# jianing-sun/Mask-YOLO

Hardware: AMD Instinct MI355X
Metric: images/sec fwd+bwd, 224x224 Shapes batch 32, at 1 MI355X (higher is better)
Workload: dtype f32

## Files before the change

### mask-yolo_amd/csrc/gemm_kernels.hip

```cpp
#include "myolo_common.h"

typedef float f32x16 __attribute__((ext_vector_type(16)));

#define BM 128
#define BN 128
#define BK 16
#define LDAS (BM + 2)

enum { AM_PLAIN = 0, AM_CONV3 = 1, AM_DECONV = 2 };
enum { EP_PLAIN = 0, EP_DECONV = 1, EP_DECONV_MASK = 2 };

struct GemmArgs {
    const float* A;
    const float* B;
    float* C;
    const float* bias;
    const float* scale;
    const float* shift;
    long long M;
    int N;
    int K;
    long long lda, ldb, ldc;
    int H, W;
    int Cc;
// ... 717 lines not shown

    const int lr = tid >> 5, c4 = (tid & 31) * 4;
    const int ka = ka0 + c4;
    const bool ka_ok = ka < p.K;
    int tap = 0, c0 = ka;
    if (AMODE != AM_PLAIN) { tap = ka / p.Cc; c0 = ka - tap * p.Cc; }
    const int ty = tap / 3, tx = tap - ty * 3;
    const int ky = tap >> 1, kx = tap & 1;

    long long a_base, a_end, a_row_elems;
    if (AMODE == AM_PLAIN) { a_base = ms; a_end = me; a_row_elems = p.lda; }
    else if (AMODE == AM_CONV3) {
        a_base = ms - (p.W + 1); if (a_base < 0) a_base = 0;
        a_end = me + p.W + 1; if (a_end > p.M) a_end = p.M;
        a_row_elems = p.Cc;
    } else {
        a_base = 4 * ms - 2 * p.W; if (a_base < 0) a_base = 0;
        a_end = 4 * me + 2 * p.W + 2; if (a_end > 4 * p.M) a_end = 4 * p.M;
        a_row_elems = p.Cc;
    }
    const __amdgpu_buffer_rsrc_t ra_desc = make_rsrc(p.A + a_base * a_row_elems, (a_end - a_base) * a_row_elems * 4);
    const __amdgpu_buffer_rsrc_t rb_desc = make_rsrc(p.B + ms * p.ldb, (me - ms) * p.ldb * 4);
    const bool bcol_ok = (n0 + c4) < p.N;

    long long mrow[2];
    int ry[2], rx[2];
    unsigned alin[2], blin[2];
    const unsigned a_step = (unsigned)(BK * a_row_elems) * 4u * (AMODE == AM_DECONV ? 4u : 1u);
    const unsigned b_step = (unsigned)(BK * p.ldb) * 4u;
    const unsigned two_cc = (unsigned)(2 * a_row_elems) * 4u;
    long long tapshift = 0;
    if (AMODE == AM_CONV3) tapshift = (long long)(ty - 1) * p.W + (tx - 1);
    if (AMODE == AM_DECONV) tapshift = (long long)ky * 2 * p.W + kx;
#pragma unroll
    for (int i = 0; i < 2; ++i) {
        mrow[i] = ms + lr + 8 * i;
        ry[i] = 0; rx[i] = 0;
        if (AMODE != AM_PLAIN) {
            const long long mm = mrow[i] < p.M ? mrow[i] : 0;
            const long long n_img = mm / hw;
            const int rem = (int)(mm - n_img * hw);
            ry[i] = rem / p.W;
            rx[i] = rem - ry[i] * p.W;
        }
        if (AMODE == AM_PLAIN) alin[i] = (unsigned)((mrow[i] - a_base) * a_row_elems + ka) * 4u;
        else if (AMODE == AM_CONV3) alin[i] = (unsigned)((mrow[i] + tapshift - a_base) * a_row_elems + c0) * 4u;
        else alin[i] = (unsigned)((4 * mrow[i] + tapshift - a_base) * a_row_elems + c0) * 4u;
        blin[i] = (unsigned)((mrow[i] - ms) * p.ldb + n0 + c4) * 4u;
    }

    f32x16 acc[2][2];
#pragma unroll
    for (int t = 0; t < 2; ++t)
#pragma unroll
        for (int u = 0; u < 2; ++u)
#pragma unroll
            for (int r = 0; r < 16; ++r) acc[t][u][r] = 0.f;

    float4 ra[2], rb[2];
    bool rav[2] = {false, false};
    float4 tsc = make_float4(1.f, 1.f, 1.f, 1.f), tsh = make_float4(0.f, 0.f, 0.f, 0.f);
    if (AMODE == AM_PLAIN && p.a_scale && ka_ok) { tsc = ld4(p.a_scale + ka); tsh = ld4(p.a_shift + ka); }
    auto gload = [&]() {
#pragma unroll
        for (int i = 0; i < 2; ++i) {
            const bool mv = mrow[i] < me;
            rav[i] = mv && ka_ok;
            unsigned aoff = OOB_OFF;
            if (AMODE == AM_PLAIN) {
                if (mv && ka_ok) aoff = alin[i];
            } else if (AMODE == AM_CONV3) {
                const bool v = mv && ka_ok && (unsigned)(ry[i] + ty - 1) < (unsigned)p.H && (unsigned)(rx[i] + tx - 1) < (unsigned)p.W;
                if (v) aoff = alin[i];
            } else {
                if (mv && ka_ok) aoff = alin[i] - (unsigned)rx[i] * two_cc;
            }
            ra[i] = bufld4(ra_desc, aoff);
            rb[i] = bufld4(rb_desc, (mv && bcol_ok) ? blin[i] : OOB_OFF);
            mrow[i] += BK;
            alin[i] += a_step;
            blin[i] += b_step;
            if (AMODE != AM_PLAIN) {
                int nx = rx[i] + BK;
                const int w2 = (nx >= 2 * p.W) ? 2 : ((nx >= p.W) ? 1 : 0);
                nx -= w2 * p.W;
                int ny = ry[i] + w2;
                ny = (ny >= p.H) ? ny - p.H : ny;
                rx[i] = nx; ry[i] = ny;
            }
        }
    };
    auto sstore = [&](int buf) {
        if (AMODE == AM_PLAIN && p.a_scale) {
#pragma unroll
            for (int i = 0; i < 2; ++i)
                if (rav[i]) {
                    ra[i].x = gemm_act(fmaf(ra[i].x, tsc.x, tsh.x), p.a_act); ra[i].y = gemm_act(fmaf(ra[i].y, tsc.y, tsh.y), p.a_act);
                    ra[i].z = gemm_act(fmaf(ra[i].z, tsc.z, tsh.z), p.a_act); ra[i].w = gemm_act(fmaf(ra[i].w, tsc.w, tsh.w), p.a_act);
                }
        }
#pragma unroll
        for (int i = 0; i < 2; ++i) {
            *reinterpret_cast<float4*>(&As[buf][lr + 8 * i][c4]) = ra[i];
            *reinterpret_cast<float4*>(&Bs[buf][lr + 8 * i][c4]) = rb[i];
        }
    };

    const long long nsteps = (me > ms) ? (me - ms + BK - 1) / BK : 0;
    const int half = lane >> 5, l31 = lane & 31;
    const int arow_l = wm * 64 + l31, bcol_l = wn * 64 + l31;
    if (nsteps > 0) {
        gload();
        sstore(0);
        __syncthreads();
        int cur = 0;
        for (long long st = 0; st < nsteps; ++st) {
            const bool more = st + 1 < nsteps;
            if (more) gload();
            float fa0 = As[cur][half * 8][arow_l], fa1 = As[cur][half * 8][arow_l + 32];
            float fb0 = Bs[cur][half * 8][bcol_l], fb1 = Bs[cur][half * 8][bcol_l + 32];
#pragma unroll
            for (int j = 0; j < 8; ++j) {
                float na0 = 0.f, na1 = 0.f, nb0 = 0.f, nb1 = 0.f;
                if (j < 7) {
                    const int kk = half * 8 + j + 1;
                    na0 = As[cur][kk][arow_l]; na1 = As[cur][kk][arow_l + 32];
                    nb0 = Bs[cur][kk][bcol_l]; nb1 = Bs[cur][kk][bcol_l + 32];
                }
                MFMA_STEP()
                if (j == 3 && more) sstore(cur ^ 1);
                fa0 = na0; fa1 = na1; fb0 = nb0; fb1 = nb1;
            }
            __syncthreads();
            cur ^= 1;
        }
    }
    const int nb = p.batch > 1 ? p.batch : 1;
    float* Cp = p.C + ((long long)blockIdx.y * nb + blockIdx.z) * p.K * p.N;
#pragma unroll
    for (int t = 0; t < 2; ++t)
#pragma unroll
        for (int r = 0; r < 16; ++r) {
            const int row = ka0 + wm * 64 + t * 32 + (r & 3) + 8 * (r >> 2) + 4 * half;
            if (row >= p.K) continue;
#pragma unroll
            for (int u = 0; u < 2; ++u) {
                const int col = n0 + wn * 64 + u * 32 + l31;
                if (col < p.N) Cp[(long long)row * p.N + col] = acc[t][u][r];
            }
        }
}

template <int KT, int NT>
__global__ __launch_bounds__(256) void pw_wgrad_thin(const float* __restrict__ x, const float* __restrict__ dy, float* __restrict__ part,
                                                     long long M, int Cin, int Cout, const float* __restrict__ a_scale,
                                                     const float* __restrict__ a_shift, int a_act)
{
    __shared__ float red[4][32 * 32];
    const int lane = threadIdx.x & 63, wave = threadIdx.x >> 6;
    const int half = lane >> 5, l31 = lane & 31;
    f32x16 acc[KT][NT];
#pragma unroll
    for (int a = 0; a < KT; ++a)
#pragma unroll
        for (int b = 0; b < NT; ++b)
#pragma unroll
            for (int r = 0; r < 16; ++r) acc[a][b][r] = 0.f;
    float xs[KT], xt[KT];
#pragma unroll
    for (int a = 0; a < KT; ++a) { xs[a] = a_scale ? a_scale[32 * a + l31] : 1.f; xt[a] = a_scale ? a_shift[32 * a + l31] : 0.f; }
    const long long nwaves = (long long)gridDim.x * 4;
    const long long w0 = (long long)blockIdx.x * 4 + wave;
    constexpr int RS = (KT + NT <= 3) ? 8 : 4;
    for (long long m0 = w0 * (2 * RS); m0 < M; m0 += nwaves * (2 * RS)) {
        float xa[RS][KT], yb[RS][NT];
#pragma unroll
        for (int st = 0; st < RS; ++st) {
            const long long m = m0 + 2 * st + half;
            const bool ok = m < M;
#pragma unroll
            for (int a = 0; a < KT; ++a) {
                float v = ok ? x[m * Cin + 32 * a + l31] : 0.f;
                if (a_scale && ok) v = gemm_act(fmaf(v, xs[a], xt[a]), a_act);
                xa[st][a] = v;
            }
#pragma unroll
            for (int b = 0; b < NT; ++b) yb[st][b] = ok ? dy[m * Cout + 32 * b + l31] : 0.f;
        }
#pragma unroll
        for (int st = 0; st < RS; ++st)
#pragma unroll
            for (int a = 0; a < KT; ++a)
#pragma unroll
                for (int b = 0; b < NT; ++b)
                    acc[a][b] = __builtin_amdgcn_mfma_f32_32x32x2f32(xa[st][a], yb[st][b], acc[a][b], 0, 0, 0);
    }
    float* dst = part + (long long)blockIdx.x * Cin * Cout;
#pragma unroll
    for (int a = 0; a < KT; ++a)
#pragma unroll
        for (int b = 0; b < NT; ++b) {
            __syncthreads();
#pragma unroll
            for (int r = 0; r < 16; ++r) red[wave][((r & 3) + 8 * (r >> 2) + 4 * half) * 32 + l31] = acc[a][b][r];
            __syncthreads();
            for (int e = threadIdx.x; e < 1024; e += 256) {
                const float v = (red[0][e] + red[1][e]) + (red[2][e] + red[3][e]);
                dst[(long long)(32 * a + (e >> 5)) * Cout + 32 * b + (e & 31)] = v;
            }
        }
}

__global__ __launch_bounds__(256) void partial_sum_small(const float* __restrict__ part, float* __restrict__ out, int n, int splits)
{
    __shared__ float red[4][64];
    const int e = blockIdx.x * 64 + (threadIdx.x & 63), sl = threadIdx.x >> 6;
    float s[8] = {0.f, 0.f, 0.f, 0.f, 0.f, 0.f, 0.f, 0.f};
    if (e < n) {
        int k = sl;
        for (; k + 28 < splits; k += 32) {
#pragma unroll
            for (int u = 0; u < 8; ++u) s[u] += part[(long long)(k + 4 * u) * n + e];
        }
        for (; k < splits; k += 4) s[0] += part[(long long)k * n + e];
    }
    red[sl][threadIdx.x & 63] = ((s[0] + s[1]) + (s[2] + s[3])) + ((s[4] + s[5]) + (s[6] + s[7]));
    __syncthreads();
    if (sl == 0 && e < n) out[e] = (red[0][threadIdx.x] + red[1][threadIdx.x]) + (red[2][threadIdx.x] + red[3][threadIdx.x]);
}

__global__ __launch_bounds__(256) void splitk_reduce(const float* __restrict__ part, float* __restrict__ out, long long n, int splits)
{
    const long long n4 = (n & 3) ? 0 : (n >> 2);
    long long i = (long long)blockIdx.x * blockDim.x + threadIdx.x;
    const long long stride = (long long)gridDim.x * blockDim.x;
    const float4* p4 = reinterpret_cast<const float4*>(part);
    for (; i < n4; i += stride) {
        float4 s = make_float4(0.f, 0.f, 0.f, 0.f);
        int k = 0;
        for (; k + 4 <= splits; k += 4) {
            const float4 a = p4[(long long)(k + 0) * n4 + i], b = p4[(long long)(k + 1) * n4 + i];
            const float4 c = p4[(long long)(k + 2) * n4 + i], d = p4[(long long)(k + 3) * n4 + i];
            s.x += a.x; s.y += a.y; s.z += a.z; s.w += a.w;
            s.x += b.x; s.y += b.y; s.z += b.z; s.w += b.w;
            s.x += c.x; s.y += c.y; s.z += c.z; s.w += c.w;
            s.x += d.x; s.y += d.y; s.z += d.z; s.w += d.w;
        }
        for (; k < splits; ++k) {
            const float4 a = p4[(long long)k * n4 + i];
            s.x += a.x; s.y += a.y; s.z += a.z; s.w += a.w;
        }
        reinterpret_cast<float4*>(out)[i] = s;
    }
    for (long long j = (n4 << 2) + (long long)blockIdx.x * blockDim.x + threadIdx.x; j < n; j += stride) {
        float t = 0.f;
        for (int k = 0; k < splits; ++k) t += part[(long long)k * n + j];
        out[j] = t;
    }
}

template <int EPI>
__global__ __launch_bounds__(256) void splitk_epilogue(GemmArgs p)
{
    const long long total = p.M * (long long)(p.N >> 2);
    long long i = (long long)blockIdx.x * blockDim.x + threadIdx.x;
    const long long stride = (long long)gridDim.x * blockDim.x;
    const int nq = p.N >> 2;
    const long long slab = p.M * (long long)p.N;
    const long long hw = (long long)p.H * p.W;
    for (; i < total; i += stride) {
        const long long row = i / nq;
        const int col = (int)(i - row * nq) * 4;
        float4 s = make_float4(0.f, 0.f, 0.f, 0.f);
        for (int k = 0; k < p.ksplits; ++k) {
            const float4 a = *reinterpret_cast<const float4*>(p.part + k * slab + row * p.N + col);
            s.x += a.x; s.y += a.y; s.z += a.z; s.w += a.w;
        }
        float v[4] = {s.x, s.y, s.z, s.w};
        int tap = 0, cc = col;
        if (EPI == EP_DECONV) { tap = col / p.Co; cc = col - tap * p.Co; }
#pragma unroll
        for (int e = 0; e < 4; ++e) {
            if (p.bias) v[e] += p.bias[cc + e];
            if (p.scale) { float cs, ct; col_affine(p, col + e, cs, ct); v[e] = fmaf(v[e], cs, ct); }
            v[e] = gemm_act(v[e], p.act);
        }
        float* dst;
        if (EPI == EP_PLAIN) {
            dst = p.C + row * p.ldc + col;
        } else {
            const long long n_img = row / hw;
            const int rem = (int)(row - n_img * hw);
            const int y = rem / p.W, x = rem - y * p.W;
            dst = p.C + (n_img * 4 * hw + (long long)y * 4 * p.W + 2 * x + (long long)(tap >> 1) * 2 * p.W + (tap & 1)) * p.Co + cc;
        }
        *reinterpret_cast<float4*>(dst) = make_float4(v[0], v[1], v[2], v[3]);
    }
}

__global__ void transpose_batched(const float* __restrict__ in, float* __restrict__ out, int R, int C, int nz, int reverse)
{
    __shared__ float tile[32][33];
    const int z = blockIdx.z;
    const int zi = reverse ? (nz - 1 - z) : z;
    const float* ip = in + (long long)zi * R * C;
    float* op = out + (long long)z * R * C;
    const int c0 = blockIdx.x * 32, r0 = blockIdx.y * 32;
    for (int i = threadIdx.y; i < 32; i += blockDim.y) {
        const int r = r0 + i, c = c0 + threadIdx.x;
        tile[i][threadIdx.x] = (r < R && c < C) ? ip[(long long)r * C + c] : 0.f;
    }
    __syncthreads();
    for (int i = threadIdx.y; i < 32; i += blockDim.y) {
        const int c = c0 + i, r = r0 + threadIdx.x;
        if (r < R && c < C) op[(long long)c * R + r] = tile[threadIdx.x][i];
    }
}

__global__ __launch_bounds__(256) void deconv_mask_finish(const float* __restrict__ part, const float* __restrict__ b2,
                                                          float* __restrict__ out, long long npix, int ncls, int nslabs)
{
    const long long total = npix * ncls;
    for (long long i = (long long)blockIdx.x * blockDim.x + threadIdx.x; i < total; i += (long long)gridDim.x * blockDim.x) {
        float sacc = b2[(int)(i % ncls)];
        for (int k = 0; k < nslabs; ++k) sacc += part[(long long)k * total + i];
        out[i] = 1.f / (1.f + expf(-sacc));
    }
}

static int launch_transpose(const float* in, float* out, int R, int C, int nz, int reverse, hipStream_t s)
{
    dim3 grid((C + 31) / 32, (R + 31) / 32, nz), block(32, 8);
    hipLaunchKernelGGL(transpose_batched, grid, block, 0, s, in, out, R, C, nz, reverse);
    return 0;
}

static inline long long pw_x6_min_rows() { return g_myolo_opt.pw_x6_min_rows > 0 ? g_myolo_opt.pw_x6_min_rows : 4096; }

template <int AMODE, int EPI>
static int launch_nn(const GemmArgs& a, hipStream_t s, void* sk_ws = nullptr, size_t sk_ws_bytes = 0, long long sk_max_tiles = 512,
                     int* path = nullptr)
{
    if (path) *path = 0;
    const long long tiles = cdiv64(a.M, BM) * ((a.N + BN - 1) / BN);
    if (tiles <= 0) return MYOLO_OK;
    const bool aligned = (a.N & 3) == 0 && (a.ldb & 3) == 0 && ((uintptr_t)a.A & 15) == 0 && ((uintptr_t)a.B & 15) == 0;
    const bool kfast = (AMODE == AM_PLAIN) ? ((a.K % BK) == 0 && (a.lda & 3) == 0) : ((a.Cc % BK) == 0);
    GemmArgs& am = const_cast<GemmArgs&>(a);
    am.nt = (long long)a.M * a.N * 4 > (64ll << 20);
    if (aligned && kfast && !g_myolo_opt.gemm_generic) {
        const int nk = a.K / BK;
        int splits = 1;
        if (sk_ws && tiles < sk_max_tiles && nk >= 16 && (a.N & 3) == 0 && (EPI == EP_PLAIN ? (a.ldc & 3) == 0 : (a.Co & 3) == 0) &&
            !g_myolo_opt.no_splitk) {
            splits = (int)(1024 / tiles);
            if (splits > nk / 8) splits = nk / 8;
            const size_t per = (size_t)a.M * a.N * sizeof(float);
            if ((size_t)splits * per > sk_ws_bytes) splits = (int)(sk_ws_bytes / per);
            if (splits < 2) splits = 1;
        }
        if (path) *path = splits > 1 ? splits : 1;
        if (splits > 1) {
            am.ksplits = splits;
// ... 442 lines not shown
}

static bool pw_fwd_thin_ok(long long M, int Cin, int Cout)
{
    return (Cin == 32 || Cin == 64) && Cout == 64 && M >= 8192 && !g_myolo_opt.no_trunk_fusion;
}

static int pw_fwd_thin_wgs(long long M)
{
    long long wgs = ((M + 31) / 32 + 3) / 4;
    if (wgs > 2048) wgs = 2048;
    return (int)wgs;
}

static void pw_fwd_thin_launch(const float* x, const float* in_scale, const float* in_shift, int in_act, const float* w, float* y, double* stat,
                               long long M, int Cin, int Cout, hipStream_t s, const float* o_scale = nullptr, const float* o_shift = nullptr,
                               int o_act = MYOLO_ACT_NONE)
{
    const unsigned wgs = (unsigned)pw_fwd_thin_wgs(M);
    size_t lds = (size_t)Cout * (Cin + 4) * sizeof(float);
    if (lds < (size_t)8 * Cout * sizeof(double)) lds = (size_t)8 * Cout * sizeof(double);
#define PWT(NU_, NJ_) hipLaunchKernelGGL((pw_fwd_thin_kernel<NU_, NJ_>), dim3(wgs), dim3(256), lds, s, x, w, y, stat, M, in_scale, in_shift, in_act, o_scale, o_shift, o_act)
    if (Cin == 32) PWT(2, 4);
    else PWT(2, 8);
#undef PWT
}

static bool pw_bwd_data_thin_ok(long long M, int Cin, int Cout)
{
    return (Cin == 32 || Cin == 64) && Cout <= 256 && (Cout % 8) == 0 && M >= 8192;
}


extern "C" {

int myolo_pwconv1x1_fwd(const float* x, const float* w, const float* bias, float* y,
                        int64_t M, int Cin, int Cout, void* ws, size_t ws_bytes, void* stream)
{
    MYOLO_REQUIRE(x && w && y && M > 0 && Cin > 0 && Cout > 0, "pwconv1x1_fwd: bad arguments");
    GemmArgs a = {};
    a.A = x; a.B = w; a.C = y; a.bias = bias; a.M = M; a.N = Cout; a.K = Cin;
    a.lda = Cin; a.ldb = Cout; a.ldc = Cout; a.act = MYOLO_ACT_NONE;
    if (Cout <= 64 && (Cout & 3) != 0 && (Cin & 15) == 0 && ((uintptr_t)x & 15) == 0 && !g_myolo_opt.gemm_generic) {
        if (Cin >= 512 && (Cin & 63) == 0)
            hipLaunchKernelGGL(pw_skinny_fwd_kernel<16>, dim3((unsigned)cdiv64(M, 4)), dim3(1024), 0, (hipStream_t)stream, x, w, bias, y, (long long)M, Cin, Cout);
        else
            hipLaunchKernelGGL(pw_skinny_fwd_kernel<4>, dim3((unsigned)cdiv64(M, 4)), dim3(256), 0, (hipStream_t)stream, x, w, bias, y, (long long)M, Cin, Cout);
        MYOLO_CHECK_LAUNCH();
        return MYOLO_OK;
    }
    if (!bias && pw_fwd_thin_ok(M, Cin, Cout) && (((uintptr_t)x | (uintptr_t)w | (uintptr_t)y) & 15) == 0 && !g_myolo_opt.gemm_generic) {
        pw_fwd_thin_launch(x, nullptr, nullptr, MYOLO_ACT_NONE, w, y, nullptr, M, Cin, Cout, (hipStream_t)stream);
        MYOLO_CHECK_LAUNCH();
        return MYOLO_OK;
    }
    if (pw_smallm_ok(a)) {
        pw_smallm_launch(a, (hipStream_t)stream);
        MYOLO_CHECK_LAUNCH();
        return MYOLO_OK;
    }
    launch_nn<AM_PLAIN, EP_PLAIN>(a, (hipStream_t)stream, ws, ws_bytes, 128);
    MYOLO_CHECK_LAUNCH();
    return MYOLO_OK;
}

int myolo_pwconv1x1_affine_act_fwd(const float* x, const float* w, const float* scale, const float* shift, int act, float* y,
                                   int64_t M, int Cin, int Cout, void* ws, size_t ws_bytes, void* stream)
{
    MYOLO_REQUIRE(x && w && y && scale && shift && M > 0 && Cin > 0 && Cout > 0, "pwconv1x1_affine_act_fwd: bad arguments");
    GemmArgs a = {};
    a.A = x; a.B = w; a.C = y; a.M = M; a.N = Cout; a.K = Cin;
    a.lda = Cin; a.ldb = Cout; a.ldc = Cout; a.act = act;
    a.scale = scale; a.shift = shift;
    if (pw_fwd_thin_ok(M, Cin, Cout) && (((uintptr_t)x | (uintptr_t)w | (uintptr_t)y) & 15) == 0 && !g_myolo_opt.gemm_generic) {
        pw_fwd_thin_launch(x, nullptr, nullptr, MYOLO_ACT_NONE, w, y, nullptr, M, Cin, Cout, (hipStream_t)stream, scale, shift, act);
        MYOLO_CHECK_LAUNCH();
        return MYOLO_OK;
    }
    if (pw_smallm_ok(a)) {
        pw_smallm_launch(a, (hipStream_t)stream);
        MYOLO_CHECK_LAUNCH();
        return MYOLO_OK;
    }
    launch_nn<AM_PLAIN, EP_PLAIN>(a, (hipStream_t)stream, ws, ws_bytes, 128);
    MYOLO_CHECK_LAUNCH();
    return MYOLO_OK;
}

int myolo_pwconv1x1_bwd_data(const float* dy, const float* w, float* dx,
                             int64_t M, int Cin, int Cout, void* ws, size_t ws_bytes, void* stream)
{
    MYOLO_REQUIRE(dy && w && dx && M > 0, "pwconv1x1_bwd_data: bad arguments");
    if (pw_bwd_data_thin_ok(M, Cin, Cout) && (((uintptr_t)dy | (uintptr_t)w | (uintptr_t)dx) & 15) == 0) {
        long long wgs = ((M + 31) / 32 + 3) / 4;
        if (wgs > 4096) wgs = 4096;
        hipStream_t st = (hipStream_t)stream;
        if (Cin == 32) hipLaunchKernelGGL(pw_bwd_data_thin_kernel<1>, dim3((unsigned)wgs), dim3(256), 0, st, dy, w, dx, (long long)M, Cout, Cin);
        else hipLaunchKernelGGL(pw_bwd_data_thin_kernel<2>, dim3((unsigned)wgs), dim3(256), 0, st, dy, w, dx, (long long)M, Cout, Cin);
        MYOLO_CHECK_LAUNCH();
        return MYOLO_OK;
    }
    MYOLO_NEED_WS((size_t)Cin * Cout * sizeof(float));
    hipStream_t s = (hipStream_t)stream;
    if (g_myolo_opt.wino_x6 && !g_myolo_opt.pw_no_x6 && (Cin % 256) == 0 && (Cout % 16) == 0 && M >= pw_x6_min_rows() &&
        ws_bytes >= myolo_matmul_f32_ws_bytes(Cout, Cin, 1, MYOLO_PRODUCTS_BF16X6) && (((uintptr_t)dy | (uintptr_t)w | (uintptr_t)dx) & 15) == 0) {
        return myolo_matmul_f32_impl(dy, w, dx, M, Cout, Cin, 1, MYOLO_PRODUCTS_BF16X6, ws, ws_bytes, stream, true);
    }
    const float* wt = (const float*)myolo_wprep_resolve(w, WP_TRANSPOSE, Cin, Cout, 10, (size_t)Cin * Cout * sizeof(float), ws, s,
                                                        [=](void* d, hipStream_t st) { launch_transpose(w, (float*)d, Cin, Cout, 1, 0, st); });
    GemmArgs a = {};
    a.A = dy; a.B = wt; a.C = dx; a.M = M; a.N = Cin; a.K = Cout;
    a.lda = Cout; a.ldb = Cin; a.ldc = Cin;
    const size_t wbytes = align256((size_t)Cin * Cout * sizeof(float));
    if (pw_smallm_ok(a)) {
        pw_smallm_launch(a, s);
        MYOLO_CHECK_LAUNCH();
        return MYOLO_OK;
    }
    launch_nn<AM_PLAIN, EP_PLAIN>(a, s, (char*)ws + wbytes, ws_bytes > wbytes ? ws_bytes - wbytes : 0);
    MYOLO_CHECK_LAUNCH();
    return MYOLO_OK;
}

static int pw_bwd_weight_impl(const float* x, const float* in_scale, const float* in_shift, int in_act, const float* dy, float* dw,
                              int64_t M, int Cin, int Cout, void* ws, size_t ws_bytes, void* stream);

int myolo_pwconv1x1_bwd_weight(const float* x, const float* dy, float* dw,
                               int64_t M, int Cin, int Cout, void* ws, size_t ws_bytes, void* stream)
{
    return pw_bwd_weight_impl(x, nullptr, nullptr, MYOLO_ACT_NONE, dy, dw, M, Cin, Cout, ws, ws_bytes, stream);
}

int myolo_pwconv1x1_bwd_weight_affine_in(const float* x, const float* in_scale, const float* in_shift, int in_act, const float* dy, float* dw,
                                         int64_t M, int Cin, int Cout, void* ws, size_t ws_bytes, void* stream)
{
    MYOLO_REQUIRE(in_scale && in_shift && (Cin & 3) == 0 && (Cout & 3) == 0 &&
                  (((uintptr_t)x | (uintptr_t)dy | (uintptr_t)in_scale | (uintptr_t)in_shift) & 15) == 0 && !g_myolo_opt.gemm_generic,
                  "pwconv1x1_bwd_weight_affine_in: needs in_scale / in_shift, Cin %% 4 == 0, Cout %% 4 == 0, 16-byte aligned operands and coefficients");
    return pw_bwd_weight_impl(x, in_scale, in_shift, in_act, dy, dw, M, Cin, Cout, ws, ws_bytes, stream);
}

}

static int pw_bwd_weight_impl(const float* x, const float* in_scale, const float* in_shift, int in_act, const float* dy, float* dw,
                              int64_t M, int Cin, int Cout, void* ws, size_t ws_bytes, void* stream)
{
    MYOLO_REQUIRE(x && dy && dw && M > 0, "pwconv1x1_bwd_weight: bad arguments");
    if ((Cin == 32 || Cin == 64) && (Cout == 64 || Cout == 128) && M >= 16384 && !g_myolo_opt.gemm_generic) {
        const int nblk = M >= 300000 ? 512 : 256;
        const size_t need = (size_t)nblk * Cin * Cout * sizeof(float);
        if (ws && need <= ws_bytes) {
            hipStream_t s = (hipStream_t)stream;
            float* part = (float*)ws;
#define THIN(KT_, NT_) hipLaunchKernelGGL((pw_wgrad_thin<KT_, NT_>), dim3(nblk), dim3(256), 0, s, x, dy, part, (long long)M, Cin, Cout, in_scale, in_shift, in_act)
            if (Cin == 32 && Cout == 64) THIN(1, 2);
            else if (Cin == 32 && Cout == 128) THIN(1, 4);
            else if (Cin == 64 && Cout == 64) THIN(2, 2);
            else THIN(2, 4);
#undef THIN
            const int n = Cin * Cout;
            hipLaunchKernelGGL(partial_sum_small, dim3((unsigned)((n + 63) / 64)), dim3(256), 0, s, (const float*)part, dw, n, nblk);
            MYOLO_CHECK_LAUNCH();
            return MYOLO_OK;
        }
    }
    if (g_myolo_opt.wino_x6 && !g_myolo_opt.pw_no_x6 && myolo_gemm_tn_x6_ok(Cin, Cout) && M >= pw_x6_min_rows() && (((uintptr_t)x | (uintptr_t)dy | (uintptr_t)dw) & 15) == 0) {
        const long long rows[1] = {M}, off[1] = {0};
        const int nq[1] = {1};
        if (myolo_gemm_tn_x6_ws_bytes(1, rows, nq, Cin, Cout) <= ws_bytes && ws) {
            const int rc = myolo_gemm_tn_x6_runs(x, dy, dw, 1, rows, off, off, nq, Cin, Cout, ws, ws_bytes, (hipStream_t)stream, in_scale, in_shift, in_act);
            if (rc) return rc;
            MYOLO_CHECK_LAUNCH();
            return MYOLO_OK;
        }
    }
    GemmArgs a = {};
    a.A = x; a.B = dy; a.M = M; a.N = Cout; a.K = Cin; a.lda = Cin; a.ldb = Cout;
    a.a_scale = in_scale; a.a_shift = in_shift; a.a_act = in_act;
    int rc = launch_tn<AM_PLAIN>(a, dw, ws, ws_bytes, (hipStream_t)stream, "pwconv1x1_bwd_weight");
    if (rc) return rc;
    MYOLO_CHECK_LAUNCH();
    return MYOLO_OK;
}

extern "C" {

int myolo_pwconv1x1_bnstats_ok(int Cin, int Cout) { return (Cin % BK) == 0 && (Cout & 3) == 0 && !g_myolo_opt.gemm_generic ? 1 : 0; }

static size_t pw_split_bytes(int64_t M, int Cout)
{
    const long long tiles = cdiv64(M, BM) * ((Cout + BN - 1) / BN);
    return tiles < 128 ? align256((size_t)8 * M * Cout * sizeof(float)) : 0;
}

size_t myolo_pwconv1x1_bnstats_ws_bytes(int64_t M, int Cin, int Cout)
{
    const size_t tiles = (size_t)cdiv64(M, BM);
    const size_t fused = align256(tiles * 2 * Cout * sizeof(double)) + align256(2 * Cout * sizeof(double)) +
                         ((Cin >= 128 && (Cout % 256) == 0) ? myolo_pw_x6_split_bytes(Cin, Cout) : 0);
    const size_t split = pw_split_bytes(M, Cout) + align256((size_t)1024 * 2 * Cout * sizeof(double)) + align256(2 * Cout * sizeof(double));
    return fused > split ? fused : split;
}

}

int myolo_bn_stats_launch(const float* x, const float* gamma, const float* beta, float* mean, float* var, float* scale, float* shift,
                          float* moving_mean, float* moving_var, long long M, int C, void* ws, size_t ws_bytes, hipStream_t s);

extern "C" {

int myolo_pwconv1x1_bnstats_fwd(const float* x, const float* in_scale, const float* in_shift, int in_act, const float* w, float* y,
                                const float* gamma, const float* beta, float* mean, float* var, float* scale, float* shift,
                                float* moving_mean, float* moving_var, int64_t M, int Cin, int Cout, int phases, void* ws, size_t ws_bytes, void* stream)
{
    MYOLO_REQUIRE(x && w && y && gamma && beta && mean && var && scale && shift && M > 0 && !in_scale == !in_shift && (phases & 3) != 0, "pwconv1x1_bnstats_fwd: bad arguments");
    MYOLO_REQUIRE(myolo_pwconv1x1_bnstats_ok(Cin, Cout) && ((uintptr_t)x & 15) == 0 && ((uintptr_t)w & 15) == 0 && ((uintptr_t)y & 15) == 0,
                  "pwconv1x1_bnstats_fwd: needs Cin %% 16 == 0, Cout %% 4 == 0 and 16-byte aligned operands");
    MYOLO_NEED_WS(myolo_pwconv1x1_bnstats_ws_bytes(M, Cin, Cout));
    hipStream_t s = (hipStream_t)stream;
    if (in_scale && (((uintptr_t)in_scale | (uintptr_t)in_shift) & 15) != 0) {
        const size_t coef = align256((size_t)Cin * sizeof(float));
        const size_t need = myolo_pwconv1x1_bnstats_ws_bytes(M, Cin, Cout) + 2 * coef + 256;
        if (ws_bytes < need) { myolo_set_error("pwconv1x1_bnstats_fwd: unaligned in_scale / in_shift need %zu bytes of workspace (%zu given)", need, ws_bytes); return MYOLO_EWORKSPACE; }
        float* cs = (float*)(((uintptr_t)ws + ws_bytes - 2 * coef) & ~(uintptr_t)255);
        (void)hipMemcpyAsync(cs, in_scale, (size_t)Cin * sizeof(float), hipMemcpyDeviceToDevice, s);
        (void)hipMemcpyAsync((char*)cs + coef, in_shift, (size_t)Cin * sizeof(float), hipMemcpyDeviceToDevice, s);
        in_scale = cs; in_shift = (const float*)((char*)cs + coef);
        ws_bytes = (size_t)((char*)cs - (char*)ws);
    }
    GemmArgs a = {};
    a.A = x; a.B = w; a.C = y; a.M = M; a.N = Cout; a.K = Cin;
    a.lda = Cin; a.ldb = Cout; a.ldc = Cout; a.act = MYOLO_ACT_NONE;
    a.a_scale = in_scale; a.a_shift = in_shift; a.a_act = in_act;
    const int tiles = (int)cdiv64(M, BM);
    const size_t pbytes = align256((size_t)tiles * 2 * Cout * sizeof(double));
    double* part = (double*)ws;
    double* tot = (double*)((char*)ws + pbytes);
    if (myolo_pw_x6_ok(Cin, Cout) && M >= pw_x6_min_rows() && !g_myolo_opt.no_trunk_fusion) {
        void* split = (char*)ws + pbytes + align256(2 * Cout * sizeof(double));
        if (phases & 1) myolo_pw_x6_fwd(x, in_scale, in_shift, in_act, w, y, part, M, Cin, Cout, split, s);
        MYOLO_CHECK_LAUNCH();
        if (phases & 2) myolo_bn_stats_from_partials(part, tot, tiles, Cout, (double)M, gamma, beta, mean, var, scale, shift, moving_mean, moving_var, s);
        MYOLO_CHECK_LAUNCH();
        return MYOLO_OK;
    }
    if (pw_fwd_thin_ok(M, Cin, Cout)) {
        const int wgs = pw_fwd_thin_wgs(M);
        if (phases & 1) pw_fwd_thin_launch(x, in_scale, in_shift, in_act, w, y, part, M, Cin, Cout, s);
        MYOLO_CHECK_LAUNCH();
        if (phases & 2) myolo_bn_stats_from_partials(part, tot, wgs, Cout, (double)M, gamma, beta, mean, var, scale, shift, moving_mean, moving_var, s);
        MYOLO_CHECK_LAUNCH();
        return MYOLO_OK;
    }
    if (pw_smallm_ok(a)) {
        if (phases & 1) pw_smallm_launch(a, s);
        MYOLO_CHECK_LAUNCH();
        if (!(phases & 2)) return MYOLO_OK;
        return myolo_bn_stats_launch(y, gamma, beta, mean, var, scale, shift, moving_mean, moving_var, M, Cout, ws, ws_bytes, s);
    }
    a.stat = g_myolo_opt.no_trunk_fusion ? nullptr : part;
    const size_t skb = pw_split_bytes(M, Cout);
    const long long otiles = cdiv64(M, BM) * ((Cout + BN - 1) / BN);
    const int nkt = Cin / BK;
    const bool one_pass = !(skb != 0 && !g_myolo_opt.no_splitk && nkt >= 16 && otiles < 128 && (1024 / otiles >= 2) && nkt / 8 >= 2);
    if (phases & 1) {
        int path = 0;
        launch_nn<AM_PLAIN, EP_PLAIN>(a, s, skb ? ws : nullptr, skb, 128, &path);
        MYOLO_CHECK_LAUNCH();
        if ((path == 1) != one_pass && path != 0) { myolo_set_error("pwconv1x1_bnstats_fwd: launcher path %d disagrees with the planned one", path); return MYOLO_EINVAL; }
    }
    if (!(phases & 2)) return MYOLO_OK;
    if (one_pass && !g_myolo_opt.no_trunk_fusion) {
        myolo_bn_stats_from_partials(part, tot, tiles, Cout, (double)M, gamma, beta, mean, var, scale, shift, moving_mean, moving_var, s);
        MYOLO_CHECK_LAUNCH();
        return MYOLO_OK;
    }
    return myolo_bn_stats_launch(y, gamma, beta, mean, var, scale, shift, moving_mean, moving_var, M, Cout, (char*)ws + skb, ws_bytes - skb, s);
}

int myolo_conv3x3_fwd(const float* x, const float* w, const float* bias, float* y,
                      int N, int H, int W, int Cin, int Cout, void* ws, size_t ws_bytes, void* stream)
{
    MYOLO_REQUIRE(x && w && y && N > 0 && H > 0 && W > 0, "conv3x3_fwd: bad arguments");
    MYOLO_REQUIRE(Cin % BK == 0, "conv3x3_fwd: Cin must be a multiple of %d (got %d)", BK, Cin);
    GemmArgs a = {};
    a.A = x; a.B = w; a.C = y; a.bias = bias; a.M = (long long)N * H * W; a.N = Cout; a.K = 9 * Cin;
    a.ldb = Cout; a.ldc = Cout; a.H = H; a.W = W; a.Cc = Cin;
    launch_nn<AM_CONV3, EP_PLAIN>(a, (hipStream_t)stream, ws, ws_bytes);
    MYOLO_CHECK_LAUNCH();
    return MYOLO_OK;
}

int myolo_conv3x3_affine_act_fwd(const float* x, const float* w, const float* bias, const float* scale, const float* shift,
                                 float* y, int N, int H, int W, int Cin, int Cout, int act, void* ws, size_t ws_bytes, void* stream)
{
    MYOLO_REQUIRE(x && w && y && scale && shift && N > 0 && H > 0 && W > 0, "conv3x3_affine_act_fwd: bad arguments");
    MYOLO_REQUIRE(Cin % BK == 0, "conv3x3_affine_act_fwd: Cin must be a multiple of %d (got %d)", BK, Cin);
    MYOLO_REQUIRE(act == MYOLO_ACT_NONE || act == MYOLO_ACT_RELU, "conv3x3_affine_act_fwd: act must be NONE or RELU");
    GemmArgs a = {};
    a.A = x; a.B = w; a.C = y; a.bias = bias; a.scale = scale; a.shift = shift; a.act = act;
    a.M = (long long)N * H * W; a.N = Cout; a.K = 9 * Cin;
    a.ldb = Cout; a.ldc = Cout; a.H = H; a.W = W; a.Cc = Cin;
    launch_nn<AM_CONV3, EP_PLAIN>(a, (hipStream_t)stream, ws, ws_bytes);
    MYOLO_CHECK_LAUNCH();
    return MYOLO_OK;
}

// ... 166 lines not shown
```

### mask-yolo_amd/csrc/mem_kernels.hip

```cpp
#include "myolo_common.h"
#include <type_traits>
#include <stdlib.h>
#include <stdarg.h>
#include <string.h>

static thread_local char g_err[512] = "";
extern "C" void myolo_set_error(const char* fmt, ...)
{
    va_list ap;
    va_start(ap, fmt);
    vsnprintf(g_err, sizeof(g_err), fmt, ap);
    va_end(ap);
}
extern "C" const char* myolo_last_error_string(void) { return g_err; }
extern "C" int myolo_version(void) { return 213; }

static MyoloOptions default_options() { MyoloOptions o = {}; o.bn_fused_tf_variance = 1; o.tn_wgs = 224; return o; }
MyoloOptions g_myolo_opt = default_options();
static int* option_slot(const char* name)
{
    static const struct { const char* n; int MyoloOptions::*m; } tab[] = {
        {"gemm_generic", &MyoloOptions::gemm_generic}, {"no_splitk", &MyoloOptions::no_splitk}, {"bf16_no256", &MyoloOptions::bf16_no256},
        {"bf16_force256", &MyoloOptions::bf16_force256}, {"bf16_no_c3", &MyoloOptions::bf16_no_c3}, {"bf16_no_loopn", &MyoloOptions::bf16_no_loopn},
        {"bf16_mask_valu", &MyoloOptions::bf16_mask_valu}, {"bf16_mask_nofin", &MyoloOptions::bf16_mask_nofin},
        {"deconv_mask_legacy", &MyoloOptions::deconv_mask_legacy}, {"crop_bf16_legacy", &MyoloOptions::crop_bf16_legacy},
        {"tune0", &MyoloOptions::tune0}, {"wino_x6", &MyoloOptions::wino_x6}, {"wino_no_bt", &MyoloOptions::wino_no_bt},
        {"wino_no_mixed", &MyoloOptions::wino_no_mixed}, {"x6_no_half_tiles", &MyoloOptions::x6_no_half_tiles},
        {"w63_legacy", &MyoloOptions::w63_legacy}, {"pw_x6_min_rows", &MyoloOptions::pw_x6_min_rows}, {"deconv_no_x6", &MyoloOptions::deconv_no_x6},
        {"pw_no_smallm", &MyoloOptions::pw_no_smallm}, {"pw_no_x6", &MyoloOptions::pw_no_x6}, {"tn_no_x6", &MyoloOptions::tn_no_x6},
        {"tn_wgs", &MyoloOptions::tn_wgs}, {"tn_x6_legacy", &MyoloOptions::tn_x6_legacy}, {"no_trunk_fusion", &MyoloOptions::no_trunk_fusion},
        {"bn_fused_tf_variance", &MyoloOptions::bn_fused_tf_variance},
    };
    if (!name) return nullptr;
    for (const auto& e : tab)
        if (strcmp(e.n, name) == 0) return &(g_myolo_opt.*(e.m));
    return nullptr;
}
extern "C" int myolo_set_option(const char* name, int value)
{
    int* s = option_slot(name);
    MYOLO_REQUIRE(s, "set_option: unknown option '%s'", name ? name : "(null)");
    *s = value;
    return MYOLO_OK;
}
extern "C" int myolo_get_option(const char* name, int* value)
{
    int* s = option_slot(name);
    MYOLO_REQUIRE(s && value, "get_option: unknown option '%s'", name ? name : "(null)");
    *value = *s;
    return MYOLO_OK;
}

#include <vector>
struct WPrepEntry {
    const void* w; int kind; long long d0, d1, d2;
    size_t off, bytes;
    unsigned long long gen;
    unsigned long long last_use;
    std::function<void(void*, hipStream_t)> run;
};
struct WPrep {
    char* arena; size_t cap, used;
    unsigned long long gen;
    std::vector<WPrepEntry> e;
    long long hits, misses;
    long long overflows;
};
static WPrep* g_wprep = nullptr;

const void* myolo_wprep_resolve(const void* w, int kind, long long d0, long long d1, long long d2, size_t bytes, void* fallback, hipStream_t s,
                                const std::function<void(void*, hipStream_t)>& run)
{
    WPrep* r = g_wprep;
    if (r) {
        for (auto& en : r->e)
            if (en.w == w && en.kind == kind && en.d0 == d0 && en.d1 == d1 && en.d2 == d2 && en.bytes == bytes) {
                en.last_use = r->gen;
                if (en.gen == r->gen) { ++r->hits; return r->arena + en.off; }
                ++r->misses;
                run(fallback, s);
                return fallback;
            }
        const size_t need = align256(bytes);
        if (r->used + need <= r->cap) {
            r->e.push_back(WPrepEntry{w, kind, d0, d1, d2, r->used, bytes, 0ull, r->gen, run});
            r->used += need;
        } else
            ++r->overflows;
        ++r->misses;
    }
    run(fallback, s);
    return fallback;
}

extern "C" int myolo_wprep_create(void* arena, size_t arena_bytes, void** handle)
{
    MYOLO_REQUIRE(handle && arena && ((uintptr_t)arena & 255) == 0, "wprep_create: needs a 256-byte aligned device arena and a handle slot");
    WPrep* r = new WPrep();
    r->arena = (char*)arena; r->cap = arena_bytes; r->used = 0; r->gen = 1; r->hits = r->misses = r->overflows = 0;
    *handle = r;
    return MYOLO_OK;
}
extern "C" int myolo_wprep_destroy(void* h)
{
    if (g_wprep == (WPrep*)h) g_wprep = nullptr;
    delete (WPrep*)h;
    return MYOLO_OK;
}
extern "C" int myolo_wprep_activate(void* h) { g_wprep = (WPrep*)h; return MYOLO_OK; }
extern "C" int myolo_wprep_count(void* h) { return h ? (int)((WPrep*)h)->e.size() : 0; }
extern "C" int myolo_wprep_invalidate(void* h) { if (h) ++((WPrep*)h)->gen; return MYOLO_OK; }
extern "C" int myolo_wprep_stats(void* h, long long* hits, long long* misses, long long* bytes_used)
{
    MYOLO_REQUIRE(h, "wprep_stats: null registry");
    WPrep* r = (WPrep*)h;
    if (hits) *hits = r->hits;
    if (misses) *misses = r->misses;
    if (bytes_used) *bytes_used = (long long)r->used;
    return MYOLO_OK;
}
extern "C" int myolo_wprep_overflows(void* h, long long* n)
{
    MYOLO_REQUIRE(h && n, "wprep_overflows: null registry or result slot");
    *n = ((WPrep*)h)->overflows;
    return MYOLO_OK;
}
extern "C" int myolo_wprep_refresh(void* h, int first, int last, int max_idle, void* stream)
{
    if (!h) { myolo_set_error("wprep_refresh: null registry"); return -1; }
    WPrep* r = (WPrep*)h;
    if (last > (int)r->e.size()) last = (int)r->e.size();
    int n = 0;
    std::vector<const void*> bs;
    std::vector<void*> bd;
    std::vector<long long> bk, bn_, bkn;
    for (int i = first < 0 ? 0 : first; i < last; ++i) {
        WPrepEntry& en = r->e[i];
        if (max_idle > 0 && r->gen - en.last_use > (unsigned long long)max_idle) continue;
        if (en.kind == WP_X6_SPLIT) {
            bs.push_back(en.w); bd.push_back(r->arena + en.off); bk.push_back(en.d0); bn_.push_back(en.d1); bkn.push_back(en.d2);
        } else
            en.run(r->arena + en.off, (hipStream_t)stream);
        en.gen = r->gen;
        ++n;
    }
    if (!bs.empty()) myolo_x6_split_batched((int)bs.size(), bs.data(), bd.data(), bk.data(), bn_.data(), bkn.data(), (hipStream_t)stream);
    if (hipGetLastError() != hipSuccess) { myolo_set_error("wprep_refresh: a launch failed"); return -1; }
    return n;
}

__device__ __forceinline__ float4 ld4g(const float* p) { return *reinterpret_cast<const float4*>(p); }
__device__ __forceinline__ void st4g(float* p, float4 v) { *reinterpret_cast<float4*>(p) = v; }
typedef float f32x4n __attribute__((ext_vector_type(4)));
__device__ __forceinline__ void st4g_nt(float* p, float4 v)
{
    f32x4n t = {v.x, v.y, v.z, v.w};
    __builtin_nontemporal_store(t, reinterpret_cast<f32x4n*>(p));
}
__device__ __forceinline__ float4 f4zero() { return make_float4(0.f, 0.f, 0.f, 0.f); }
__device__ __forceinline__ float4 f4fma(float4 a, float4 b, float4 c)
{
    return make_float4(fmaf(a.x, b.x, c.x), fmaf(a.y, b.y, c.y), fmaf(a.z, b.z, c.z), fmaf(a.w, b.w, c.w));
}
__device__ __forceinline__ float actf(float v, int act)
{
    if (act == MYOLO_ACT_RELU) return fmaxf(v, 0.f);
    if (act == MYOLO_ACT_RELU6) return fminf(fmaxf(v, 0.f), 6.f);
    return v;
}
__device__ __forceinline__ float actmask(float v, int act)
{
    if (act == MYOLO_ACT_RELU) return v > 0.f ? 1.f : 0.f;
    if (act == MYOLO_ACT_RELU6) return (v > 0.f && v < 6.f) ? 1.f : 0.f;
    return 1.f;
}

struct ColGeom {
    int cl;
    int pl;
    int cgroups;
    int rblocks;
    long long rows_per_block;
};
// ... 3319 lines not shown
```

### mask-yolo_amd/csrc/myolo_common.h

```cpp
#pragma once
#include <hip/hip_runtime.h>
#include <stdint.h>
#include <stdio.h>
#include "../../include/myolo_hip_internal.h"

extern "C" void myolo_set_error(const char* fmt, ...);

struct MyoloOptions {
    int gemm_generic;
    int no_splitk;
    int bf16_no256;
    int bf16_no_loopn;
    int bf16_mask_valu;
    int bf16_mask_nofin;
    int deconv_mask_legacy;
    int bf16_no_c3;
    int bf16_force256;
    int crop_bf16_legacy;
    int tune0;
    int wino_x6;
    int wino_no_bt;
    int wino_no_mixed;
    int x6_no_half_tiles;
    int w63_legacy;
    int pw_x6_min_rows;
    int deconv_no_x6;
    int pw_no_smallm;
    int pw_no_x6;
    int tn_no_x6;
    int tn_wgs;
    int tn_x6_legacy;
    int no_trunk_fusion;
    int bn_fused_tf_variance;
};
extern MyoloOptions g_myolo_opt;

#define MYOLO_REQUIRE(cond, ...)                                   \
    do {                                                           \
        if (!(cond)) {                                             \
            myolo_set_error(__VA_ARGS__);                          \
            return MYOLO_EINVAL;                                   \
        }                                                          \
    } while (0)

#define MYOLO_NEED_WS(bytes)                                                         \
    do {                                                                             \
        if ((size_t)(bytes) > ws_bytes || (ws == nullptr && (bytes) > 0)) {          \
            myolo_set_error("%s: workspace too small (%zu needed, %zu given)",       \
                            __func__, (size_t)(bytes), ws_bytes);                    \
            return MYOLO_EWORKSPACE;                                                 \
        }                                                                            \
    } while (0)

#define MYOLO_CHECK_LAUNCH()                                                         \
    do {                                                                             \
        hipError_t e__ = hipGetLastError();                                          \
        if (e__ != hipSuccess) {                                                     \
            myolo_set_error("%s: launch failed: %s", __func__, hipGetErrorString(e__)); \
            return MYOLO_ELAUNCH;                                                    \
        }                                                                            \
    } while (0)

#include <functional>
enum { WP_TRANSPOSE = 1, WP_X6_SPLIT = 2, WP_WINO63_U = 3, WP_WINO43_U = 4 };
const void* myolo_wprep_resolve(const void* w, int kind, long long d0, long long d1, long long d2, size_t bytes, void* fallback, hipStream_t s,
                                const std::function<void(void*, hipStream_t)>& run);

int myolo_x6_split_batched(int n, const void* const* src, void* const* dst, const long long* K, const long long* N, const long long* kn, hipStream_t s);

static inline int64_t cdiv64(int64_t a, int64_t b) { return (a + b - 1) / b; }
static inline size_t align256(size_t x) { return (x + 255) & ~(size_t)255; }

#define BN_EPS_F 1e-3f
#define BN_MOMENTUM_F 0.99f

int myolo_gemm_nn_batched(const float* A, const float* B, float* C, long long M, int K, int N, int batch, hipStream_t s);
bool myolo_gemm_nt_batched_ok(int K, int N);
bool myolo_gemm_nt_batched_x6(int K, int N);
bool myolo_deconv_mask_mm_ok(int Cin, int Cout);
size_t myolo_deconv_mask_mm_split_bytes(int Cin, int Cout);
int myolo_deconv_mask_mm(const float* x, const float* w, const float* bias, const float* w2, float* part, void* split,
                         long long M, int H, int W, int Cin, int Cout, int ncls, hipStream_t s,
                         const int32_t* keep_inv = nullptr, float* keep_d = nullptr, int keep_cap = 0,
                         const float* b2 = nullptr, float* p_out = nullptr, int* finished = nullptr);
int myolo_gemm_nt_batched_runs(const float* A, const float* Bt, float* C, int nruns, const long long* rows, const long long* a_off,
                               const long long* b_off, const long long* c_off, const int* nq, int K, int N, hipStream_t s);
bool myolo_gemm_tn_x6_ok(int Ka, int N);
size_t myolo_gemm_tn_x6_ws_bytes(int nruns, const long long* rows, const int* nq, int Ka, int N);
int myolo_gemm_tn_x6_runs(const float* A, const float* B, float* C, int nruns, const long long* rows, const long long* a_off, const long long* b_off,
                          const int* nq, int Ka, int N, void* part, size_t part_bytes, hipStream_t s,
                          const float* a_scale = nullptr, const float* a_shift = nullptr, int a_act = 0);
bool myolo_deconv_x6_ok(int Cin, int Co, int which);
int myolo_deconv_x6_fwd(const float* x, const float* w, const float* bias, float* y, long long M, int H, int W, int Cin, int Co, int act,
                        void* split, hipStream_t s);
int myolo_deconv_x6_bwd_data(const float* dy, const float* w, float* dx, long long M, int H, int W, int Cin, int Co, void* split, hipStream_t s);
size_t myolo_deconv_x6_bwd_weight_ws_bytes(long long M, int Cin, int Co);
int myolo_deconv_x6_bwd_weight(const float* x, const float* dy, float* dw, long long M, int H, int W, int Cin, int Co, void* part, size_t part_bytes,
                               hipStream_t s);
int myolo_matmul_f32_impl(const float* A, const float* B, float* C, int64_t M, int K, int N, int b_is_nk, int products,
                          void* ws, size_t ws_bytes, void* stream, bool b_is_weight);
bool myolo_pw_x6_ok(int K, int N);
size_t myolo_pw_x6_split_bytes(int K, int N);
int myolo_pw_x6_fwd(const float* x, const float* in_scale, const float* in_shift, int in_act, const float* w, float* y, double* stat,
                    long long M, int K, int N, void* split, hipStream_t s);
size_t myolo_gemm_tn_batched_ws_bytes(long long M, int Ka, int N, int batch);
int myolo_gemm_tn_batched(const float* A, const float* B, float* C, long long M, int Ka, int N, int batch, void* ws, size_t ws_bytes,
                          hipStream_t s);
void myolo_launch_deconv_mask_finish(const float* part, const float* b2, float* out, long long npix, int ncls, int nslabs, hipStream_t s);
void myolo_bn_stats_from_partials(const double* part, double* tot, int nblk, int C, double M, const float* gamma, const float* beta,
                                  float* mean, float* var, float* scale, float* shift, float* mmean, float* mvar, hipStream_t s);
```

Measured before the change: 1660.

## Software-pipeline thin pointwise weight-gradient kernel with multi-stage register prefetch

Rewrites the thin 1x1-conv weight-gradient MFMA kernel to keep several stages of x/dy loads in flight in registers. It uses explicit vmcnt waits so global-load latency overlaps the MFMA accumulation. Out-of-range rows are clamped to a valid address and zeroed after the load, and the affine+activation is applied branch-free. Occupancy is hinted with launch_bounds(256,2). The old kernel is kept behind a legacy option. The risks are higher register pressure, and correctness that depends on the hand-computed waitcnt encoding.

New measurement: 1662 (median of 4 runs). Within noise of the previous version (+0.1%).

```diff
diff --git a/mask-yolo_amd/csrc/gemm_kernels.hip b/mask-yolo_amd/csrc/gemm_kernels.hip
--- a/mask-yolo_amd/csrc/gemm_kernels.hip
+++ b/mask-yolo_amd/csrc/gemm_kernels.hip
@@ -893,11 +893,124 @@
 }
 
 template <int KT, int NT>
-__global__ __launch_bounds__(256) void pw_wgrad_thin(const float* __restrict__ x, const float* __restrict__ dy, float* __restrict__ part,
-                                                     long long M, int Cin, int Cout, const float* __restrict__ a_scale,
-                                                     const float* __restrict__ a_shift, int a_act)
+__device__ __forceinline__ void pw_wgrad_thin_store(const f32x16 (&acc)[KT][NT], float* __restrict__ part, int Cin, int Cout)
 {
     __shared__ float red[4][32 * 32];
+    const int lane = threadIdx.x & 63, wave = threadIdx.x >> 6;
+    const int half = lane >> 5, l31 = lane & 31;
+    float* dst = part + (long long)blockIdx.x * Cin * Cout;
+#pragma unroll
+    for (int a = 0; a < KT; ++a)
+#pragma unroll
+        for (int b = 0; b < NT; ++b) {
+            __syncthreads();
+#pragma unroll
+            for (int r = 0; r < 16; ++r) red[wave][((r & 3) + 8 * (r >> 2) + 4 * half) * 32 + l31] = acc[a][b][r];
+            __syncthreads();
+            for (int e = threadIdx.x; e < 1024; e += 256) {
+                const float v = (red[0][e] + red[1][e]) + (red[2][e] + red[3][e]);
+                dst[(long long)(32 * a + (e >> 5)) * Cout + 32 * b + (e & 31)] = v;
+            }
+        }
+}
+
+template <int KT, int NT>
+__global__ __launch_bounds__(256, 2) void pw_wgrad_thin(const float* __restrict__ x, const float* __restrict__ dy, float* __restrict__ part,
+                                                        long long M, int Cin, int Cout, const float* __restrict__ a_scale,
+                                                        const float* __restrict__ a_shift, int a_act)
+{
+    const int lane = threadIdx.x & 63, wave = __builtin_amdgcn_readfirstlane(threadIdx.x >> 6);
+    const int half = lane >> 5, l31 = lane & 31;
+    f32x16 acc[KT][NT];
+#pragma unroll
+    for (int a = 0; a < KT; ++a)
+#pragma unroll
+        for (int b = 0; b < NT; ++b)
+#pragma unroll
+            for (int r = 0; r < 16; ++r) acc[a][b][r] = 0.f;
+    float xs[KT], xt[KT];
+#pragma unroll
+    for (int a = 0; a < KT; ++a) { xs[a] = a_scale ? a_scale[32 * a + l31] : 1.f; xt[a] = a_scale ? a_shift[32 * a + l31] : 0.f; }
+    constexpr int RS = (KT + NT <= 3) ? 8 : 4;
+    constexpr int LD = RS * (KT + NT);
+    constexpr int NS = 3 * LD <= 63 ? 4 : 3;
+    constexpr int CI = 32 * KT, CO = 32 * NT;
+    constexpr int WAIT_OWN = ((((NS - 2) * LD) >> 4) << 14) | 0x0f70 | (((NS - 2) * LD) & 15);
+    static_assert((NS - 1) * LD <= 63 && NS >= 2, "more loads in flight than the vmcnt counter holds");
+    const long long step = (long long)gridDim.x * 4 * (2 * RS);
+    const unsigned vx = (half * CI + l31) * 4, vy = (half * CO + l31) * 4, v0 = l31 * 4;
+    float xa[NS][RS][KT], yb[NS][RS][NT];
+    long long m0 = ((long long)blockIdx.x * 4 + wave) * (2 * RS);
+    const long long mfirst = m0 < M ? m0 : 0;
+    auto issue = [&](int s, long long mi) {
+        const int lim = mi >= M ? 0 : (int)(M - mi < 2 * RS ? M - mi : 2 * RS);
+        const long long mb = mi >= M ? mfirst : mi;
+        const char* xb = reinterpret_cast<const char*>(x) + mb * (CI * 4);
+        const char* db = reinterpret_cast<const char*>(dy) + mb * (CO * 4);
+#pragma unroll
+        for (int st = 0; st < RS; ++st) {
+            const bool ok = 2 * st + half < lim;
+            const unsigned ox = ok ? vx + st * (2 * CI * 4) : v0, oy = ok ? vy + st * (2 * CO * 4) : v0;
+#pragma unroll
+            for (int a = 0; a < KT; ++a) xa[s][st][a] = *reinterpret_cast<const float*>(xb + ox + a * 128);
+#pragma unroll
+            for (int b = 0; b < NT; ++b) yb[s][st][b] = *reinterpret_cast<const float*>(db + oy + b * 128);
+        }
+    };
+    const float act_lo = 0.f, act_hi = a_act == MYOLO_ACT_RELU6 ? 6.f : __builtin_inff();
+    const bool act_none = a_act != MYOLO_ACT_RELU && a_act != MYOLO_ACT_RELU6;
+    auto affine = [&](int s, int lim) {
+#pragma unroll
+        for (int st = 0; st < RS; ++st) {
+            const bool ok = 2 * st + half < lim;
+#pragma unroll
+            for (int a = 0; a < KT; ++a) {
+                const float v = fmaf(xa[s][st][a], xs[a], xt[a]);
+                const float r = fminf(fmaxf(v, act_lo), act_hi);
+                xa[s][st][a] = ok ? (act_none ? v : r) : 0.f;
+            }
+        }
+    };
+    auto consume = [&](int s, long long mi) {
+        const int lim = (int)(M - mi < 2 * RS ? M - mi : 2 * RS);
+        if (lim < 2 * RS) {
+#pragma unroll
+            for (int st = 0; st < RS; ++st) {
+                const bool ok = 2 * st + half < lim;
+#pragma unroll
+                for (int a = 0; a < KT; ++a) xa[s][st][a] = ok ? xa[s][st][a] : 0.f;
+#pragma unroll
+                for (int b = 0; b < NT; ++b) yb[s][st][b] = ok ? yb[s][st][b] : 0.f;
+            }
+        }
+        if (a_scale) affine(s, lim);
+#pragma unroll
+        for (int st = 0; st < RS; ++st)
+#pragma unroll
+            for (int a = 0; a < KT; ++a)
+#pragma unroll
+                for (int b = 0; b < NT; ++b)
+                    acc[a][b] = __builtin_amdgcn_mfma_f32_32x32x2f32(xa[s][st][a], yb[s][st][b], acc[a][b], 0, 0, 0);
+    };
+#pragma unroll
+    for (int s = 0; s < NS - 1; ++s) issue(s, m0 + s * step);
+    while (m0 < M) {
+#pragma unroll
+        for (int s = 0; s < NS; ++s) {
+            __builtin_amdgcn_s_waitcnt(WAIT_OWN);
+            issue((s + NS - 1) % NS, m0 + (NS - 1) * step);
+            if (m0 < M) consume(s, m0);
+            m0 += step;
+        }
+    }
+    pw_wgrad_thin_store<KT, NT>(acc, part, Cin, Cout);
+}
+
+template <int KT, int NT>
+__global__ __launch_bounds__(256) void pw_wgrad_thin_legacy(const float* __restrict__ x, const float* __restrict__ dy, float* __restrict__ part,
+                                                            long long M, int Cin, int Cout, const float* __restrict__ a_scale,
+                                                            const float* __restrict__ a_shift, int a_act)
+{
     const int lane = threadIdx.x & 63, wave = threadIdx.x >> 6;
     const int half = lane >> 5, l31 = lane & 31;
     f32x16 acc[KT][NT];
@@ -936,20 +1049,7 @@
                 for (int b = 0; b < NT; ++b)
                     acc[a][b] = __builtin_amdgcn_mfma_f32_32x32x2f32(xa[st][a], yb[st][b], acc[a][b], 0, 0, 0);
     }
-    float* dst = part + (long long)blockIdx.x * Cin * Cout;
-#pragma unroll
-    for (int a = 0; a < KT; ++a)
-#pragma unroll
-        for (int b = 0; b < NT; ++b) {
-            __syncthreads();
-#pragma unroll
-            for (int r = 0; r < 16; ++r) red[wave][((r & 3) + 8 * (r >> 2) + 4 * half) * 32 + l31] = acc[a][b][r];
-            __syncthreads();
-            for (int e = threadIdx.x; e < 1024; e += 256) {
-                const float v = (red[0][e] + red[1][e]) + (red[2][e] + red[3][e]);
-                dst[(long long)(32 * a + (e >> 5)) * Cout + 32 * b + (e & 31)] = v;
-            }
-        }
+    pw_wgrad_thin_store<KT, NT>(acc, part, Cin, Cout);
 }
 
 __global__ __launch_bounds__(256) void partial_sum_small(const float* __restrict__ part, float* __restrict__ out, int n, int splits)
@@ -1698,7 +1798,13 @@
         if (ws && need <= ws_bytes) {
             hipStream_t s = (hipStream_t)stream;
             float* part = (float*)ws;
-#define THIN(KT_, NT_) hipLaunchKernelGGL((pw_wgrad_thin<KT_, NT_>), dim3(nblk), dim3(256), 0, s, x, dy, part, (long long)M, Cin, Cout, in_scale, in_shift, in_act)
+#define THIN(KT_, NT_)                                                                                                                                    \
+    do {                                                                                                                                                  \
+        if (g_myolo_opt.pw_wgrad_thin_legacy)                                                                                                             \
+            hipLaunchKernelGGL((pw_wgrad_thin_legacy<KT_, NT_>), dim3(nblk), dim3(256), 0, s, x, dy, part, (long long)M, Cin, Cout, in_scale, in_shift, in_act); \
+        else                                                                                                                                              \
+            hipLaunchKernelGGL((pw_wgrad_thin<KT_, NT_>), dim3(nblk), dim3(256), 0, s, x, dy, part, (long long)M, Cin, Cout, in_scale, in_shift, in_act); \
+    } while (0)
             if (Cin == 32 && Cout == 64) THIN(1, 2);
             else if (Cin == 32 && Cout == 128) THIN(1, 4);
             else if (Cin == 64 && Cout == 64) THIN(2, 2);
diff --git a/mask-yolo_amd/csrc/mem_kernels.hip b/mask-yolo_amd/csrc/mem_kernels.hip
--- a/mask-yolo_amd/csrc/mem_kernels.hip
+++ b/mask-yolo_amd/csrc/mem_kernels.hip
@@ -28,7 +28,8 @@
         {"wino_no_mixed", &MyoloOptions::wino_no_mixed}, {"x6_no_half_tiles", &MyoloOptions::x6_no_half_tiles},
         {"w63_legacy", &MyoloOptions::w63_legacy}, {"pw_x6_min_rows", &MyoloOptions::pw_x6_min_rows}, {"deconv_no_x6", &MyoloOptions::deconv_no_x6},
         {"pw_no_smallm", &MyoloOptions::pw_no_smallm}, {"pw_no_x6", &MyoloOptions::pw_no_x6}, {"tn_no_x6", &MyoloOptions::tn_no_x6},
-        {"tn_wgs", &MyoloOptions::tn_wgs}, {"tn_x6_legacy", &MyoloOptions::tn_x6_legacy}, {"no_trunk_fusion", &MyoloOptions::no_trunk_fusion},
+        {"tn_wgs", &MyoloOptions::tn_wgs}, {"tn_x6_legacy", &MyoloOptions::tn_x6_legacy},
+        {"pw_wgrad_thin_legacy", &MyoloOptions::pw_wgrad_thin_legacy}, {"no_trunk_fusion", &MyoloOptions::no_trunk_fusion},
         {"bn_fused_tf_variance", &MyoloOptions::bn_fused_tf_variance},
     };
     if (!name) return nullptr;
diff --git a/mask-yolo_amd/csrc/myolo_common.h b/mask-yolo_amd/csrc/myolo_common.h
--- a/mask-yolo_amd/csrc/myolo_common.h
+++ b/mask-yolo_amd/csrc/myolo_common.h
@@ -30,6 +30,7 @@
     int tn_no_x6;
     int tn_wgs;
     int tn_x6_legacy;
+    int pw_wgrad_thin_legacy;
     int no_trunk_fusion;
     int bn_fused_tf_variance;
 };
```
